# jhidalgocarrio/slam-localization

Hardware: NVIDIA B200
Metric: filter-steps/sec (predict+update) (higher is better)
Workload: dtype f64

## Files before the change

slam-localization_b200/csrc/slb_predict12.cuh:

```cuda
#pragma once
#include "slb_internal.h"
#include "slb_models.cuh"
#include "slb_ptx.cuh"

namespace slbd {

template <int N_>
struct CycCfg {
    static constexpr int N = N_;
    static constexpr int RT = (N_ + 3) / 4;
    static constexpr int CT = (N_ + 7) / 8;
    SLB_HD static constexpr int cb(int k) { return k * N_ - k * (k - 1) / 2; }
    SLB_HD static constexpr bool exists(int r, int c) { return 4 * r < N_ && 8 * c < N_ && 4 * r + 3 >= 8 * c; }
    SLB_HD static constexpr bool live(int k, int r, int c) { return exists(r, c) && 8 * c + 7 > k && 4 * r + 3 > k; }
    SLB_HD static constexpr bool row_live(int k, int r) {
        for (int c = 0; c < CT; ++c)
            if (live(k, r, c)) return true;
        return false;
    }
    SLB_HD static constexpr bool col_live(int k, int c) {
        for (int r = 0; r < RT; ++r)
            if (live(k, r, c)) return true;
        return false;
    }
};

template <class C, int K>
struct CholStep {
    template <class Tile>
    SLB_DEV static void run(Tile &T, double *Ls, int a_, int b_, bool &ok, double x, double nrcp) {
        constexpr int N = C::N, RT = C::RT, CT = C::CT;
        constexpr int rk = K >> 2, bk = K & 7, ck = K >> 3;
        constexpr int K1 = K + 1 < N ? K + 1 : K;
        constexpr int owner1 = (K1 & 3) + 4 * (K1 & 7);
        constexpr int base = C::cb(K) - K;
        ok = ok && (x > 0.0);
        const double xn_old = __shfl_sync(FULL, T[K1 >> 2][K1 >> 3], owner1);
#pragma unroll
        for (int r = rk; r < RT; ++r) {
            const int i = a_ + 4 * r;
            if (b_ == bk && i >= K && i < N) Ls[base + i] = T[r][ck];
        }
        __syncwarp();
        double li[RT], lj[CT];
#pragma unroll
        for (int r = 0; r < RT; ++r)
            if (C::row_live(K, r)) li[r] = Ls[base + a_ + 4 * r];
#pragma unroll
        for (int c = 0; c < CT; ++c)
            if (C::col_live(K, c)) lj[c] = Ls[base + b_ + 8 * c] * nrcp;
        double xn = x, nrcpn = nrcp;
        if (K + 1 < N) {
            const double u1 = Ls[base + K + 1];
            xn = fma(u1, u1 * nrcp, xn_old);
            nrcpn = -rcp_fast(xn);
        }
#pragma unroll
        for (int r = 0; r < RT; ++r)
#pragma unroll
            for (int c = 0; c < CT; ++c)
                if (C::live(K, r, c)) T[r][c] = fma(li[r], lj[c], T[r][c]);
        CholStep<C, K + 1>::run(T, Ls, a_, b_, ok, xn, nrcpn);
    }
};
template <class C>
struct CholStep<C, C::N> {
    template <class Tile>
    SLB_DEV static void run(Tile &, double *, int, int, bool &, double, double) {}
};

constexpr int PRED_DS = 20;
constexpr int PRED_LS = 78 + 16;
constexpr int PRED_D = 28 * PRED_DS;
constexpr int PRED_W = 144;
constexpr int PRED_FK = 12 * PRED_DS;
constexpr int PRED_RSD = 16;
constexpr int PRED_SLOTS = 16;
constexpr int PRED_SCR = PRED_LS + PRED_D + PRED_W + PRED_FK + PRED_RSD + PRED_SLOTS;
constexpr int PRED_PR = 520;
constexpr int PRED_PF = 8 * 12;
constexpr int PRED_MU = 26;
constexpr int PRED_SM = PRED_PR + PRED_PF + PRED_SCR + PRED_MU + 2;
static_assert(16 * PRED_SM * 8 <= 227 * 1024, "two CTAs of 8 warps per SM");

SLB_DEV void load_q_entries(const double *Qi, int a_, int b_, double *qv) {
    const int rr[6] = {b_, b_, 8 + b_, 8 + b_, 8 + b_, 8 + b_};
    const int cc[6] = {2 * a_, 2 * a_ + 1, 2 * a_, 2 * a_ + 1, 8 + 2 * a_, 9 + 2 * a_};
#pragma unroll
    for (int k = 0; k < 6; ++k) qv[k] = (rr[k] < 12 && cc[k] <= rr[k]) ? __ldg(Qi + rr[k] * 12 + cc[k]) : 0.0;
}

SLB_DEV void warp_sum12(const double *v, double *out, double *slots, int lane) {
    double a[8], b[4], c[2], d1;
    const bool h16 = lane & 16, h8 = lane & 8, h4 = lane & 4, h2 = lane & 2;
#pragma unroll
    for (int i = 0; i < 8; ++i) {
        const double lo = v[i], hi = i < 4 ? v[8 + i] : 0.0;
        const double r = __shfl_xor_sync(FULL, h16 ? lo : hi, 16);
        a[i] = (h16 ? hi : lo) + r;
    }
#pragma unroll
    for (int i = 0; i < 4; ++i) {
        const double r = __shfl_xor_sync(FULL, h8 ? a[i] : a[4 + i], 8);
        b[i] = (h8 ? a[4 + i] : a[i]) + r;
    }
#pragma unroll
    for (int i = 0; i < 2; ++i) {
        const double r = __shfl_xor_sync(FULL, h4 ? b[i] : b[2 + i], 4);
        c[i] = (h4 ? b[2 + i] : b[i]) + r;
    }
    {
        const double r = __shfl_xor_sync(FULL, h2 ? c[0] : c[1], 2);
        d1 = (h2 ? c[1] : c[0]) + r;
    }
    d1 += __shfl_xor_sync(FULL, d1, 1);
    const int idx = (h16 ? 8 : 0) + (h8 ? 4 : 0) + (h4 ? 2 : 0) + (h2 ? 1 : 0);
    __syncwarp();
    if (!(lane & 1)) slots[idx] = d1;
    __syncwarp();
#pragma unroll
    for (int i = 0; i < 6; ++i) {
        const double2 t = *reinterpret_cast<const double2 *>(slots + 2 * i);
        out[2 * i] = t.x;
        out[2 * i + 1] = t.y;
    }
}

template <int PM, bool CROSS, bool PIN, class View>
SLB_DEV int predict12_block(View v, const double *mu_src, const double *u, double dt, double *scr, const double *Qg,
                            const double *qv, int nf, double *mu_dst, int lane, bool &dirty) {
    typedef LayState12 L;
    typedef CycCfg<12> C;
    constexpr int ROW0 = View::ROW0;
    double *Ls = scr, *D = Ls + PRED_LS, *W = D + PRED_D, *Fk = W + PRED_W, *rsd = Fk + PRED_FK, *slots = rsd + PRED_RSD;
    const int a_ = lane & 3, b_ = lane >> 2;
    double mu[13];
#pragma unroll
    for (int c = 0; c < 13; ++c) mu[c] = mu_src[c];
    ProcessModel<PM> f;
    f.prepare(u, dt);
    double T[C::RT][C::CT];
#pragma unroll
    for (int r = 0; r < C::RT; ++r)
#pragma unroll
        for (int c = 0; c < C::CT; ++c)
            if (C::exists(r, c)) {
                const int i = a_ + 4 * r, j = b_ + 8 * c;
                T[r][c] = (i < 12 && j <= i) ? v.at(i, ROW0 + j) : 0.0;
            }
    bool ok = true;
    {
        const double x0 = __shfl_sync(FULL, T[0][0], 0);
        CholStep<C, 0>::run(T, Ls, a_, b_, ok, x0, -rcp_fast(x0));
    }
    if (!ok) return SLB_ST_CHOL_FAIL;
    __syncwarp();
    if (lane < 12) {
        double sq_, rs_;
        sqrt_rsqrt(Ls[C::cb(lane)], sq_, rs_);
        rsd[lane] = rs_;
    }
    __syncwarp();
    const bool act = lane < 25;
    const int j = lane >= 1 ? (lane - 1) >> 1 : 0, jc = j < 12 ? j : 11;
    double Y[13];
    {
        const double sgn = (lane & 1) ? rsd[jc] : -rsd[jc];
        const int cj = C::cb(jc) - jc;
        double d[12], X[13];
#pragma unroll
        for (int r = 0; r < 12; ++r) d[r] = (act && lane >= 1 && r >= jc) ? sgn * Ls[cj + r] : 0.0;
        boxplus<L>(mu, d, 1.0, X);
        f.apply(X, Y);
    }
    double ref[13];
#pragma unroll
    for (int c = 0; c < 13; ++c) ref[c] = bcast(Y[c], 0);
    int it = 0;
    double nrm2;
    do {
        double dd[12], md[12], nr[13];
        boxminus<L>(Y, ref, dd);
#pragma unroll
        for (int r = 0; r < 12; ++r) dd[r] = act ? dd[r] : 0.0;
        warp_sum12(dd, md, slots, lane);
        nrm2 = 0.0;
#pragma unroll
        for (int r = 0; r < 12; ++r) {
            md[r] *= (1.0 / 25.0);
            nrm2 += md[r] * md[r];
        }
        boxplus<L>(ref, md, 1.0, nr);
#pragma unroll
        for (int c = 0; c < 13; ++c) ref[c] = nr[c];
    } while (sqrt(nrm2) > 1e-6 && ++it < 10000);
    int st = (it >= 10000) ? SLB_ST_MEAN_NOCONV : 0;
    {
        double dY[12];
        boxminus<L>(Y, ref, dY);
        if (lane < 28) {
#pragma unroll
            for (int r = 0; r < 12; r += 2)
                *reinterpret_cast<double2 *>(D + lane * PRED_DS + r) = act ? make_double2(dY[r], dY[r + 1]) : make_double2(0.0, 0.0);
        }
    }
    __syncwarp();
    dirty = true;
    {
        double c00[2] = {0.0, 0.0}, c10[2] = {0.0, 0.0}, c11[2] = {0.0, 0.0};
        const double *p0 = D + a_ * PRED_DS + b_, *p1 = p0 + 8;
#pragma unroll
        for (int k0 = 0; k0 < 28; k0 += 4) {
            const double f0 = p0[k0 * PRED_DS], f1 = p1[k0 * PRED_DS];
            dmma884(c00[0], c00[1], f0, f0);
            dmma884(c10[0], c10[1], f1, f0);
            dmma884(c11[0], c11[1], f1, f1);
        }
        if (CROSS) {
            for (int e = lane; e < 144; e += 32) {
                const int jj = e / 12, c = e - jj * 12;
                W[e] = 0.5 * (D[(1 + 2 * jj) * PRED_DS + c] - D[(2 + 2 * jj) * PRED_DS + c]);
            }
            __syncwarp();
        }
        auto put = [&](int r, int c, double x, int k) {
            if (r < 12 && c <= r) v.at(r, ROW0 + c) = 0.5 * x + (PIN ? qv[k] : __ldg(Qg + r * 12 + c));
        };
        const int r = b_, c = 2 * a_;
        put(r, c, c00[0], 0); put(r, c + 1, c00[1], 1);
        put(8 + r, c, c10[0], 2); put(8 + r, c + 1, c10[1], 3);
        put(8 + r, 8 + c, c11[0], 4); put(8 + r, 8 + c + 1, c11[1], 5);
    }
    if constexpr (CROSS) {
        if (lane < 12) {
            double x[12];
#pragma unroll
            for (int r = 11; r >= 0; --r) {
                double sacc = 0.0;
#pragma unroll
                for (int p = r + 1; p < 12; ++p) sacc = fma(Ls[C::cb(r) - r + p], x[p], sacc);
                const double rs = rsd[r];
                x[r] = (W[r * 12 + lane] - rs * sacc) * rs;
            }
#pragma unroll
            for (int r = 0; r < 12; ++r) Fk[lane * PRED_DS + r] = x[r];
        }
        __syncwarp();
        double oc[2][3][2];
        {
            const int r0 = min(b_, 11), r1 = min(8 + b_, 11);
#pragma unroll
            for (int I = 0; I < 2; ++I)
#pragma unroll
                for (int J = 0; J < 3; ++J) oc[I][J][0] = oc[I][J][1] = 0.0;
#pragma unroll
            for (int k0 = 0; k0 < 12; k0 += 4) {
                const double fa0 = Fk[r0 * PRED_DS + k0 + a_], fa1 = Fk[r1 * PRED_DS + k0 + a_];
#pragma unroll
                for (int J = 0; J < 3; ++J) {
                    const double bv = v.at(k0 + a_, 8 * J + b_);
                    dmma884(oc[0][J][0], oc[0][J][1], fa0, bv);
                    dmma884(oc[1][J][0], oc[1][J][1], fa1, bv);
                }
            }
        }
        const int nft = (nf + 7) >> 3;
        double of[4][2][2];
        {
            const int c0 = min(b_, 11), c1 = min(8 + b_, 11);
#pragma unroll
            for (int I = 0; I < 4; ++I) {
                if (I < nft) {
                    of[I][0][0] = of[I][0][1] = of[I][1][0] = of[I][1][1] = 0.0;
                    const int fr = min(8 * I + b_, nf - 1);
#pragma unroll
                    for (int k0 = 0; k0 < 12; k0 += 4) {
                        const double av = v.feat(fr, k0 + a_);
                        dmma884(of[I][0][0], of[I][0][1], av, Fk[c0 * PRED_DS + k0 + a_]);
                        dmma884(of[I][1][0], of[I][1][1], av, Fk[c1 * PRED_DS + k0 + a_]);
                    }
                }
            }
        }
        __syncwarp();
#pragma unroll
        for (int I = 0; I < 2; ++I)
#pragma unroll
            for (int J = 0; J < 3; ++J)
                if (8 * I + b_ < 12)
                    *reinterpret_cast<double2 *>(v.P + v.idx(8 * I, 8 * J) + 2 * lane) = make_double2(oc[I][J][0], oc[I][J][1]);
#pragma unroll
        for (int I = 0; I < 4; ++I) {
            if (I < nft) {
#pragma unroll
                for (int J = 0; J < 2; ++J) {
                    const int fr = 8 * I + b_, c = 8 * J + 2 * a_;
                    if (fr < nf && c < 12) { v.feat(fr, c) = of[I][J][0]; v.feat(fr, c + 1) = of[I][J][1]; }
                }
            }
        }
    }
    bool finite = true;
#pragma unroll
    for (int c = 0; c < 13; ++c) {
        finite = finite && isfinite(ref[c]);
        if (lane == c) mu_dst[c] = ref[c];
    }
    if (!finite) st |= SLB_ST_NONFINITE;
    __syncwarp();
    return st;
}

struct SpanView {
    static constexpr int ROW0 = 24;
    double *P, *Pf;
    int N;
    SLB_DEV int idx(int r, int c) const { return prec(N, 24 + r, c) - tri(24, 0); }
    SLB_DEV double &at(int r, int c) const { return P[idx(r, c)]; }
    SLB_DEV double &feat(int fr, int c) const { return fr < 4 ? at(12 + fr, 24 + c) : Pf[(fr - 4) * 12 + c]; }
};
template <int ROW0_>
struct PackedView {
    static constexpr int ROW0 = ROW0_;
    double *P;
    SLB_DEV int idx(int r, int c) const { return tri(ROW0 + r, c) - tri(ROW0, 0); }
    SLB_DEV double &at(int r, int c) const { return P[idx(r, c)]; }
};

template <int PM, int WPB, int ROW0, int MU0, bool CROSS, bool PIN = false>
__global__ void __launch_bounds__(WPB * 32, 2) predict12_kernel(slb::FilterArgs a) {
    extern __shared__ __align__(16) double smem[];
    const int lane = threadIdx.x & 31, w = threadIdx.x >> 5;
    const int inst = blockIdx.x * WPB + w;
    if (inst >= a.B) return;
    double *Pr = smem + (size_t)w * PRED_SM, *Pf = Pr + PRED_PR, *scr = Pf + PRED_PF;
    double *mus = scr + PRED_SCR, *us = mus + 13;
    uint64_t *bar = reinterpret_cast<uint64_t *>(mus + PRED_MU);
    static_assert(!CROSS || ROW0 == 24, "the tiled span is tile rows 3..4");
    const int nf = CROSS ? a.nk + a.nl : 0, N = CROSS ? 36 + nf : ROW0 + 12;
    constexpr int T0 = ROW0 * (ROW0 + 1) / 2, T1 = (ROW0 + 12) * (ROW0 + 13) / 2;
    constexpr int RS = CROSS ? 40 : ROW0 + 12;
    constexpr int NFS = RS - 36;
    const int SPAN = CROSS ? tri(min(N, RS), 0) - T0 : T1 - T0;
    const int nfr = CROSS && nf > NFS ? nf - NFS : 0;
    static_assert(tri(RS, 0) - T0 <= PRED_PR && (!CROSS || 12 * (48 - RS) <= PRED_PF), "row span");
    double *Pg = a.P + (size_t)inst * a.pstride;
    double *mug = a.mu + (size_t)inst * a.qstride;
    const int a_ = lane & 3, b_ = lane >> 2;

    static_assert((T0 * 8) % 16 == 0 && ((T1 - T0) * 8) % 16 == 0 && PRED_SM % 2 == 0 &&
                      (!CROSS || (((tri(RS, 0) - T0) * 8) % 16 == 0 && ((tri(39, 0) - T0) * 8) % 16 == 0)),
                  "bulk copy needs 16-byte alignment");
    if (lane == 0) {
        mbar_init(bar, 1);
        mbar_expect_tx(bar, SPAN * 8);
        bulk_g2s(Pr, Pg + T0, SPAN * 8, bar);
    }
    for (int e = lane; e < nfr * 12; e += 32) {
        const int r = e / 12, c = e - r * 12;
        cp_async8(Pf + e, Pg + prec(N, RS + r, 24 + c));
    }
    double qv[PIN ? 6 : 1];
    if (PIN) load_q_entries(a.Q + (size_t)inst * a.qs, a_, b_, qv);
    static_assert(ProcessModel<PM>::NU <= PRED_MU - 13, "control input slots");
    if (lane < 13) cp_async8(mus + lane, mug + MU0 + lane);
    if (lane < ProcessModel<PM>::NU) cp_async8(us + lane, a.u + (size_t)inst * ProcessModel<PM>::NU + lane);
    cp_async_wait_all();
    __syncwarp();
    mbar_wait(bar, 0);

    int st;
    bool dirty = false;
    if constexpr (CROSS) st = predict12_block<PM, true, PIN>(SpanView{Pr, Pf, N}, mus, us, a.dt, scr, a.Q, qv, nf, mug + MU0, lane, dirty);
    else st = predict12_block<PM, false, PIN>(PackedView<ROW0>{Pr}, mus, us, a.dt, scr, a.Q, qv, nf, mug + MU0, lane, dirty);
    if (dirty) {
        for (int e = lane; e < SPAN; e += 32) Pg[T0 + e] = Pr[e];
        for (int e = lane; e < nfr * 12; e += 32) {
            const int r = e / 12, c = e - r * 12;
            Pg[prec(N, RS + r, 24 + c)] = Pf[e];
        }
    }
    if (st && lane == 0) a.status[inst] |= st;
}

}
```

slam-localization_b200/csrc/slb_usckf_step.cuh:

```cuda
#pragma once
#include "slb_predict12.cuh"

#ifndef SLB_USCKF_CTA_SYNC
#define SLB_USCKF_CTA_SYNC 0
#endif
#if SLB_USCKF_CTA_SYNC
#define SLB_CTA_SYNC() __syncthreads()
#else
#define SLB_CTA_SYNC() ((void)0)
#endif

namespace slbd {

template <int NK_, int NL_>
struct StepCfg {
    static constexpr int NK = NK_, NL = NL_, NF = NK_ + NL_;
    static constexpr int N = 36 + NK_ + NL_;
    static constexpr int NP = N * (N + 1) / 2;
    static constexpr int PSTR = (NP + 15) / 16 * 16;
    static constexpr int QD = 39 + NK_ + NL_;
    static constexpr int QS = (QD + 1) / 2 * 2;
    static constexpr int NT = (N + 7) / 8;
    static constexpr int NPAD = 8 * NT;
    static constexpr int JM = 36 + NK_;
    static constexpr int NPAN = (JM + 3) / 4;
    static constexpr int NCOL = 4 * NPAN;
    static constexpr int JLAST = (NCOL - 1) >> 3;
    static constexpr int NGRP = (NPAN + 3) / 4;
    static constexpr int PL = 2 * NPAD + 8;
    static constexpr int PS4 = 2 * PL + 2;
    static constexpr int KP = (NK_ + 3) / 4 * 4;
    static constexpr int NTN = (NK_ + 7) / 8;
    static constexpr int LF = 4 * PS4;
    static constexpr int LRAW = 2 * PL;
    static constexpr int KK = 2 * NPAD * KP + NPAD;
    static constexpr int SCR0 = (LF + LRAW > KK ? LF + LRAW : KK);
    static constexpr int WS = 20;
    static constexpr int WGS = WS * NK_;
    static constexpr int UPD_SCR = SCR0 + WGS + NPAD;
    static constexpr int SCR = (UPD_SCR > PRED_SCR ? UPD_SCR : PRED_SCR);
    static constexpr int ZS = (NK_ + 1) / 2 * 2;
    static constexpr int SM = PSTR + QS + SCR + ZS + 2;
    static constexpr int RP = (NK_ * (NK_ + 1) / 2 + 1) / 2 * 2;
    static constexpr int SMP = SM + RP;
    static_assert(NK_ % 3 == 0 && NK_ >= 3, "the VO model moves 3-D features");
    static_assert(N <= 64, "two rows per lane");
    static_assert(SM % 2 == 0 && PSTR % 2 == 0 && QS % 2 == 0, "16-byte alignment of the bulk copies");
};

template <int M>
SLB_DEV bool sym_inverse(const double *S, double *Si) {
    double L[M * (M + 1) / 2], dd[M], rd[M];
    bool ok = true;
#pragma unroll
    for (int k = 0; k < M; ++k) {
        double d = S[tri(k, k)];
#pragma unroll
        for (int p = 0; p < k; ++p) d = fma(-L[tri(k, p)] * L[tri(k, p)], dd[p], d);
        ok = ok && (d > 0.0);
        dd[k] = d;
        rd[k] = rcp_fast(d);
#pragma unroll
        for (int i = k + 1; i < M; ++i) {
            double s = S[tri(i, k)];
#pragma unroll
            for (int p = 0; p < k; ++p) s = fma(-L[tri(i, p)] * L[tri(k, p)], dd[p], s);
            L[tri(i, k)] = s * rd[k];
        }
    }
    double X[M * (M + 1) / 2];
#pragma unroll
    for (int j = 0; j < M; ++j) {
        X[tri(j, j)] = 1.0;
#pragma unroll
        for (int i = j + 1; i < M; ++i) {
            double s = 0.0;
#pragma unroll
            for (int p = j; p < i; ++p) s = fma(-L[tri(i, p)], X[tri(p, j)], s);
            X[tri(i, j)] = s;
        }
    }
#pragma unroll
    for (int i = 0; i < M; ++i)
#pragma unroll
        for (int j = 0; j <= i; ++j) {
            double s = 0.0;
#pragma unroll
            for (int k = i; k < M; ++k) s = fma(X[tri(k, i)] * rd[k], X[tri(k, j)], s);
            Si[tri(i, j)] = s;
        }
    return ok;
}

template <int NK>
SLB_DEV void vo_model(const double *pk, const double *qk, const double *pi, const double *qi, const double *f, double *z) {
    double dq[4];
    quat_cmul(qi, qk, dq);
#pragma unroll
    for (int c = 0; c < NK; c += 3) {
        double rz[3];
        rotmat_apply(dq, f + c, rz);
        z[c] = rz[0] + (pk[0] - pi[0]);
        z[c + 1] = rz[1] + (pk[1] - pi[1]);
        z[c + 2] = rz[2] + (pk[2] - pi[2]);
    }
}

template <class C>
struct UpdState {
    double c0[C::NT][C::JLAST + 1], c1[C::NT][C::JLAST + 1];
    double x0[C::NT][C::NTN], x1[C::NT][C::NTN];
    double esum[C::NK], eep[C::NK * (C::NK + 1) / 2];
    double z0[C::NK];
    bool ok;
};

template <class C, int G>
SLB_DEV void sigma_group(UpdState<C> &s, const double *mus_, const double *Lf, double *Wg, const double *dv, int lane) {
    constexpr int NK = C::NK, PS4 = C::PS4;
    double mus[40 + NK];
    {
        const double2 *m2 = reinterpret_cast<const double2 *>(mus_);
#pragma unroll
        for (int e = 0; e < 4; ++e) { const double2 v = m2[e]; mus[2 * e] = v.x; mus[2 * e + 1] = v.y; }
#pragma unroll
        for (int e = 13; e < 17; ++e) { const double2 v = m2[e]; mus[2 * e] = v.x; mus[2 * e + 1] = v.y; }
#pragma unroll
        for (int c = 0; c < NK; ++c) mus[39 + c] = mus_[39 + c];
    }
    constexpr int col0 = 16 * G;
    constexpr int ncols = C::NCOL - col0 < 16 ? C::NCOL - col0 : 16;
    const bool neg = lane & 1, act = (lane >> 1) < ncols;
    const int jl = act ? lane >> 1 : 0;
    const double rs = rsqrt_fast(dv[col0 + jl]);
    const double sgn = act ? (neg ? -rs : rs) : 0.0;
    constexpr int RW = 8 * ((col0 + ncols - 1) >> 3);
    const double *col = Lf + (jl >> 2) * PS4 + ((jl & 3) >> 1) * C::PL + (jl & 1);
    auto Lc = [&](int r) -> double { return sgn * (r >= RW || r >= col0 + jl ? col[2 * r] : 0.0); };
    double xpk[3], xqk[4], xpi[3], xqi[4], xf[NK];
    if (col0 <= 5) {
#pragma unroll
        for (int c = 0; c < 3; ++c) xpk[c] = mus[c] + Lc(c);
        const double v[3] = {Lc(3), Lc(4), Lc(5)};
        const double q[4] = {mus[3], mus[4], mus[5], mus[6]};
        double e[4];
        so3_exp(v, 1.0, e);
        quat_mul(q, e, xqk);
    } else {
#pragma unroll
        for (int c = 0; c < 3; ++c) xpk[c] = mus[c];
#pragma unroll
        for (int c = 0; c < 4; ++c) xqk[c] = mus[3 + c];
    }
    if (col0 <= 29) {
#pragma unroll
        for (int c = 0; c < 3; ++c) xpi[c] = mus[26 + c] + Lc(24 + c);
        const double v[3] = {Lc(27), Lc(28), Lc(29)};
        const double q[4] = {mus[29], mus[30], mus[31], mus[32]};
        double e[4];
        so3_exp(v, 1.0, e);
        quat_mul(q, e, xqi);
    } else {
#pragma unroll
        for (int c = 0; c < 3; ++c) xpi[c] = mus[26 + c];
#pragma unroll
        for (int c = 0; c < 4; ++c) xqi[c] = mus[29 + c];
    }
#pragma unroll
    for (int c = 0; c < NK; ++c) xf[c] = mus[39 + c] + Lc(36 + c);
    double z[NK];
    vo_model<NK>(xpk, xqk, xpi, xqi, xf, z);
    double e[NK];
#pragma unroll
    for (int c = 0; c < NK; ++c) {
        e[c] = act ? z[c] - s.z0[c] : 0.0;
        s.esum[c] += e[c];
        const double zp = __shfl_xor_sync(FULL, z[c], 1);
        if (act && !neg) Wg[c * C::WS + jl] = (0.5 * rs) * (z[c] - zp);
    }
#pragma unroll
    for (int r = 0; r < NK; ++r)
#pragma unroll
        for (int c = 0; c <= r; ++c) s.eep[tri(r, c)] = fma(e[r], e[c], s.eep[tri(r, c)]);
    __syncwarp();
    const int a_ = lane & 3, b_ = lane >> 2;
#pragma unroll
    for (int qq = 0; qq < ncols / 4; ++qq) {
        const int J0 = (col0 + 4 * qq) >> 3;
        const double *fp = Lf + qq * PS4 + (a_ >> 1) * C::PL + (a_ & 1) + 2 * b_;
        double w[C::NTN];
#pragma unroll
        for (int T = 0; T < C::NTN; ++T) w[T] = 8 * T + b_ < NK ? Wg[(8 * T + b_) * C::WS + 4 * qq + a_] : 0.0;
#pragma unroll
        for (int I = J0; I < C::NT; ++I) {
            const double f = fp[16 * I];
#pragma unroll
            for (int T = 0; T < C::NTN; ++T) dmma884(s.x0[I][T], s.x1[I][T], f, w[T]);
        }
    }
}

template <class C, int P>
struct PanelStep {
    SLB_DEV static void run(UpdState<C> &s, const double *mus, double *Lf, double *Lraw, double *Wg, double *dv, int lane) {
        constexpr int NT = C::NT, JLAST = C::JLAST, PS4 = C::PS4;
        constexpr int K = 4 * P, J0 = K >> 3, H = (K >> 2) & 1, Q = P & 3;
        constexpr int I1 = (K + 4) >> 3;
        const int a_ = lane & 3, b_ = lane >> 2;
        double *Lq = Lf + Q * PS4;
        constexpr int PL = C::PL;
        if ((a_ >> 1) == H) {
#pragma unroll
            for (int I = J0; I < NT; ++I)
                *reinterpret_cast<double2 *>(Lraw + (a_ & 1) * PL + 2 * (8 * I + b_)) = make_double2(s.c0[I][J0], s.c1[I][J0]);
        }
        __syncwarp();
        double m10, m20, m30, m21, m31, m32, r0, r1, r2, r3, d0, d1, d2, d3;
        {
            const double *A = Lraw + 2 * K, *Bp = A + PL;
            const double a00 = A[0];
            const double2 a1 = *reinterpret_cast<const double2 *>(A + 2);
            const double2 a2 = *reinterpret_cast<const double2 *>(A + 4);
            const double a22 = Bp[4];
            const double2 a3 = *reinterpret_cast<const double2 *>(A + 6), a3b = *reinterpret_cast<const double2 *>(Bp + 6);
            d0 = a00;
            r0 = rcp_fast(d0);
            m10 = a1.x * r0; m20 = a2.x * r0; m30 = a3.x * r0;
            d1 = fma(-a1.x, m10, a1.y);
            const double u21 = fma(-a2.x, m10, a2.y), u31 = fma(-a3.x, m10, a3.y);
            r1 = rcp_fast(d1);
            m21 = u21 * r1; m31 = u31 * r1;
            d2 = fma(-u21, m21, fma(-a2.x, m20, a22));
            const double u32 = fma(-u31, m21, fma(-a3.x, m20, a3b.x));
            r2 = rcp_fast(d2);
            m32 = u32 * r2;
            d3 = fma(-u32, m32, fma(-u31, m31, fma(-a3.x, m30, a3b.y)));
            r3 = rcp_fast(d3);
            s.ok = s.ok && (d0 > 0.0) && (d1 > 0.0) && (d2 > 0.0) && (d3 > 0.0);
        }
        if (lane == 0) {
            *reinterpret_cast<double2 *>(dv + K) = make_double2(d0, d1);
            *reinterpret_cast<double2 *>(dv + K + 2) = make_double2(d2, d3);
        }
        constexpr int R0 = 8 * J0, NLIVE = C::NPAD - R0;
        auto finish = [&](int i) {
            const double2 x01 = *reinterpret_cast<const double2 *>(Lraw + 2 * i);
            const double2 x23 = *reinterpret_cast<const double2 *>(Lraw + PL + 2 * i);
            const double u0 = x01.x;
            const double u1 = fma(-u0, m10, x01.y);
            const double u2 = fma(-u1, m21, fma(-u0, m20, x23.x));
            const double u3 = fma(-u2, m32, fma(-u1, m31, fma(-u0, m30, x23.y)));
            double2 u01, u23;
            u01.x = i >= K ? u0 : 0.0;
            u01.y = i >= K + 1 ? u1 : 0.0;
            u23.x = i >= K + 2 ? u2 : 0.0;
            u23.y = i >= K + 3 ? u3 : 0.0;
            *reinterpret_cast<double2 *>(Lq + 2 * i) = u01;
            *reinterpret_cast<double2 *>(Lq + PL + 2 * i) = u23;
        };
        if (NLIVE >= 32 || lane < NLIVE) finish(R0 + lane);
        if (NLIVE > 32 && lane < NLIVE - 32) finish(R0 + 32 + lane);
        __syncwarp();
        if (I1 <= JLAST) {
            double f[NT];
            const double *fp = Lq + (a_ >> 1) * PL + (a_ & 1) + 2 * b_;
#pragma unroll
            for (int I = I1; I < NT; ++I) f[I] = fp[16 * I];
            const double rlo = (a_ & 1) ? r1 : r0, rhi = (a_ & 1) ? r3 : r2;
            const double nr = -((a_ & 2) ? rhi : rlo);
#pragma unroll
            for (int J = I1; J <= JLAST; ++J) {
                const double g = f[J] * nr;
#pragma unroll
                for (int I = J; I < NT; ++I) dmma884(s.c0[I][J], s.c1[I][J], f[I], g);
            }
        }
        if (Q == 3 || P == C::NPAN - 1) {
            sigma_group<C, (P >> 2)>(s, mus, Lf, Wg, dv, lane);
            SLB_CTA_SYNC();
        }
        PanelStep<C, P + 1>::run(s, mus, Lf, Lraw, Wg, dv, lane);
    }
};
template <class C>
struct PanelStep<C, C::NPAN> {
    SLB_DEV static void run(UpdState<C> &, const double *, double *, double *, double *, double *, int) {}
};

template <int NK, int NL, bool PIN = false>
SLB_DEV int usckf_update_smem(double *Ps, double *mus, double *scr, const double *zs, const double *Rs,
                              const slb::FilterArgs &a, int lane, bool &dirty, double &m2out) {
    typedef StepCfg<NK, NL> C;
    constexpr int N = C::N, NT = C::NT, NPAD = C::NPAD, JLAST = C::JLAST, KP = C::KP;
    const int a_ = lane & 3, b_ = lane >> 2;
    double *Lf = scr, *Lraw = scr + C::LF, *Ks = scr, *Cs = scr + NPAD * KP, *Wg = scr + C::SCR0, *dv = Wg + C::WGS,
           *dl = Cs + NPAD * KP;
    UpdState<C> s;
    s.ok = true;
    auto elem = [&](int i, int j) -> double {
        if (i >= N || j >= N) return i == j ? 1.0 : 0.0;
        return i >= j ? Ps[prec(N, i, j)] : Ps[prec(N, j, i)];
    };
#pragma unroll
    for (int I = 0; I < NT; ++I)
#pragma unroll
        for (int J = 0; J <= JLAST; ++J)
            if (J < I) {
                double2 v = make_double2(0.0, 0.0);
                if (8 * I + b_ < N) v = *reinterpret_cast<const double2 *>(Ps + prec(N, 8 * I, 8 * J) + 2 * lane);
                s.c0[I][J] = v.x;
                s.c1[I][J] = v.y;
            } else if (J == I) {
                const int i = 8 * I + b_, j = 8 * J + 2 * a_;
                s.c0[I][J] = elem(i, j);
                s.c1[I][J] = elem(i, j + 1);
            }
#pragma unroll
    for (int I = 0; I < NT; ++I)
#pragma unroll
        for (int T = 0; T < C::NTN; ++T) s.x0[I][T] = s.x1[I][T] = 0.0;
#pragma unroll
    for (int c = 0; c < NK; ++c) s.esum[c] = 0.0;
#pragma unroll
    for (int e = 0; e < NK * (NK + 1) / 2; ++e) s.eep[e] = 0.0;
    {
        double pk[3], qk[4], pi[3], qi[4], ft[NK];
#pragma unroll
        for (int c = 0; c < 3; ++c) { pk[c] = mus[c]; pi[c] = mus[26 + c]; }
#pragma unroll
        for (int c = 0; c < 4; ++c) { qk[c] = mus[3 + c]; qi[c] = mus[29 + c]; }
#pragma unroll
        for (int c = 0; c < NK; ++c) ft[c] = mus[39 + c];
        vo_model<NK>(pk, qk, pi, qi, ft, s.z0);
    }
    PanelStep<C, 0>::run(s, mus, Lf, Lraw, Wg, dv, lane);
    if (!s.ok) return SLB_ST_CHOL_FAIL;

    constexpr double NS = (double)(2 * N + 1);
    double ebar[NK], S[NK * (NK + 1) / 2];
    if (PIN) {
        cp_async_wait0();
        __syncwarp();
    }
    auto Rv = [&](int r, int c) { return PIN ? Rs[tri(r, c)] : __ldg(a.R + r * NK + c); };
    if (NK == 3) {
        double v[12], o[12];
#pragma unroll
        for (int c = 0; c < 3; ++c) v[c] = s.esum[c];
#pragma unroll
        for (int e = 0; e < 6; ++e) v[3 + e] = s.eep[e];
        v[9] = v[10] = v[11] = 0.0;
        warp_sum12(v, o, dv, lane);
#pragma unroll
        for (int c = 0; c < 3; ++c) ebar[c] = o[c] * (1.0 / NS);
#pragma unroll
        for (int r = 0; r < NK; ++r)
#pragma unroll
            for (int c = 0; c <= r; ++c)
                S[tri(r, c)] = 0.5 * fma(-NS * ebar[r], ebar[c], o[3 + tri(r, c)]) + Rv(r, c);
    } else {
#pragma unroll
        for (int c = 0; c < NK; ++c) ebar[c] = warp_sum(s.esum[c]) * (1.0 / NS);
#pragma unroll
        for (int r = 0; r < NK; ++r)
#pragma unroll
            for (int c = 0; c <= r; ++c)
                S[tri(r, c)] = 0.5 * fma(-NS * ebar[r], ebar[c], warp_sum(s.eep[tri(r, c)])) + Rv(r, c);
    }
    double Si[NK * (NK + 1) / 2];
    const bool sok = sym_inverse<NK>(S, Si);
    auto SiAt = [&](int r, int c) { return r >= c ? Si[tri(r, c)] : Si[tri(c, r)]; };
    cp_async_wait0();
    __syncwarp();
    double nu[NK], sn[NK], m2 = 0.0;
#pragma unroll
    for (int c = 0; c < NK; ++c) nu[c] = zs[c] - (s.z0[c] + ebar[c]);
#pragma unroll
    for (int r = 0; r < NK; ++r) {
        double t = 0.0;
#pragma unroll
        for (int c = 0; c < NK; ++c) t = fma(SiAt(r, c), nu[c], t);
        sn[r] = t;
        m2 = fma(nu[r], t, m2);
    }
    if (!sok) return SLB_ST_CHOL_FAIL;
    m2out = m2;
    if (!chi2_accept(m2, a.gate)) return SLB_ST_GATE_REJECT;
#pragma unroll
    for (int I = 0; I < NT; ++I)
#pragma unroll
        for (int T = 0; T < C::NTN; ++T)
            if (8 * T + 2 * a_ < KP)
                *reinterpret_cast<double2 *>(Cs + (8 * I + b_) * KP + 8 * T + 2 * a_) = make_double2(s.x0[I][T], s.x1[I][T]);
    __syncwarp();
    auto finish_row = [&](int i) {
        double px[NK];
#pragma unroll
        for (int c = 0; c < NK; ++c) px[c] = Cs[i * KP + c];
        double dsum = 0.0;
#pragma unroll
        for (int c = 0; c < KP; ++c) {
            double k = 0.0;
            if (c < NK) {
#pragma unroll
                for (int p = 0; p < NK; ++p) k = fma(px[p], SiAt(p, c), k);
                dsum = fma(px[c], sn[c], dsum);
            }
            Ks[i * KP + c] = k;
            Cs[i * KP + c] = c < NK ? -px[c] : 0.0;
        }
        dl[i] = dsum;
    };
    finish_row(lane);
    if (lane + 32 < NPAD) finish_row(lane + 32);
    __syncwarp();
    dirty = true;
    bool finite = true;
    if (lane < 12) {
        const int mbw = lane & 3;
        const int mqo = 13 * (lane >> 2) + (mbw == 0 ? 0 : mbw == 1 ? 3 : mbw == 2 ? 7 : 10);
        const double v[3] = {dl[3 * lane], dl[3 * lane + 1], dl[3 * lane + 2]};
        if (mbw == 1) {
            const double q[4] = {mus[mqo], mus[mqo + 1], mus[mqo + 2], mus[mqo + 3]};
            double e[4], o[4];
            so3_exp(v, 1.0, e);
            quat_mul(q, e, o);
#pragma unroll
            for (int c = 0; c < 4; ++c) { mus[mqo + c] = o[c]; finite = finite && isfinite(o[c]); }
        } else {
#pragma unroll
            for (int c = 0; c < 3; ++c) {
                const double o = mus[mqo + c] + v[c];
                mus[mqo + c] = o;
                finite = finite && isfinite(o);
            }
        }
    }
    for (int f = lane; f < NK + NL; f += 32) {
        const double o = mus[39 + f] + dl[36 + f];
        mus[39 + f] = o;
        finite = finite && isfinite(o);
    }
    {
        double fa[NT][KP / 4], fb[NT][KP / 4];
#pragma unroll
        for (int I = 0; I < NT; ++I)
#pragma unroll
            for (int kk = 0; kk < KP / 4; ++kk) {
                fa[I][kk] = Cs[(8 * I + b_) * KP + 4 * kk + a_];
                fb[I][kk] = Ks[(8 * I + b_) * KP + 4 * kk + a_];
            }
#pragma unroll
        for (int I = 0; I < NT; ++I)
#pragma unroll
            for (int J = 0; J <= I; ++J) {
                const int i = 8 * I + b_, j = 8 * J + 2 * a_;
                if (J < I) {
                    double2 *pp = reinterpret_cast<double2 *>(Ps + prec(N, 8 * I, 8 * J) + 2 * lane);
                    const bool w = i < N;
                    double2 p = w ? *pp : make_double2(0.0, 0.0);
#pragma unroll
                    for (int kk = 0; kk < KP / 4; ++kk) dmma884(p.x, p.y, fa[I][kk], fb[J][kk]);
                    if (w) *pp = p;
                } else {
                    const bool w0 = i < N && j <= i, w1 = i < N && j + 1 <= i;
                    double p0 = w0 ? Ps[prec(N, i, j)] : 0.0, p1 = w1 ? Ps[prec(N, i, j + 1)] : 0.0;
#pragma unroll
                    for (int kk = 0; kk < KP / 4; ++kk) dmma884(p0, p1, fa[I][kk], fb[J][kk]);
                    if (w0) Ps[prec(N, i, j)] = p0;
                    if (w1) Ps[prec(N, i, j + 1)] = p1;
                }
            }
    }
    return __all_sync(FULL, finite) ? 0 : SLB_ST_NONFINITE;
}

template <int N>
struct ResidentView {
    static constexpr int ROW0 = 24;
    double *P;
    SLB_DEV int idx(int r, int c) const { return prec(N, 24 + r, c); }
    SLB_DEV double &at(int r, int c) const { return P[idx(r, c)]; }
    SLB_DEV double &feat(int fr, int c) const { return P[prec(N, 36 + fr, 24 + c)]; }
};

template <int PM, int NK, int NL, bool PRED, bool UPD, int WPB, int MINB, bool PIN = false, bool NIS = false>
__global__ void __launch_bounds__(WPB * 32, MINB) usckf_step_kernel(slb::FilterArgs a) {
    typedef StepCfg<NK, NL> C;
    constexpr int SMW = PIN ? C::SMP : C::SM;
    extern __shared__ __align__(128) double smem[];
    const int lane = threadIdx.x & 31, w = threadIdx.x >> 5;
    const int inst = blockIdx.x * WPB + w;
    if (inst >= a.B) return;
    double *Ps = smem + (size_t)w * SMW, *mus = Ps + C::PSTR, *scr = mus + C::QS, *zs = scr + C::SCR;
    double *Rs = zs + C::ZS;
    uint64_t *bar = reinterpret_cast<uint64_t *>(zs + C::ZS + (PIN ? C::RP : 0));
    double *Pg = a.P + (size_t)inst * a.pstride;
    double *mug = a.mu + (size_t)inst * a.qstride;
    if (lane == 0) {
        mbar_init(bar, 1);
        mbar_expect_tx(bar, (C::PSTR + C::QS) * 8);
        bulk_g2s(Ps, Pg, C::PSTR * 8, bar);
        bulk_g2s(mus, mug, C::QS * 8, bar);
        if (a.prefetch > 0 && inst + a.prefetch < a.B) bulk_prefetch_l2(Pg + (size_t)a.prefetch * a.pstride, C::PSTR * 8);
    }
    if (UPD && lane < NK) {
        cp_async8(zs + lane, a.z + (size_t)inst * NK + lane);
        cp_async_commit();
    }
    if (PIN && UPD) {
        const double *Ri = a.R + (size_t)inst * a.rs;
        for (int e = lane; e < NK * (NK + 1) / 2; e += 32) {
            int r = (int)((sqrtf(8.0f * e + 1.0f) - 1.0f) * 0.5f);
            r += (tri(r + 1, 0) <= e) - (tri(r, 0) > e);
            cp_async8(Rs + e, Ri + r * NK + (e - tri(r, 0)));
        }
        cp_async_commit();
    }
    double qv[PIN && PRED ? 6 : 1];
    if (PIN && PRED) load_q_entries(a.Q + (size_t)inst * a.qs, lane & 3, lane >> 2, qv);
    double u[ProcessModel<PM>::NU];
    if (PRED) {
#pragma unroll
        for (int c = 0; c < ProcessModel<PM>::NU; ++c) u[c] = a.u[(size_t)inst * ProcessModel<PM>::NU + c];
    }
    __syncwarp();
    mbar_wait(bar, 0);
    SLB_CTA_SYNC();
    int st = 0;
    bool dirty = false;
    if (PRED) {
        st = predict12_block<PM, true, PIN>(ResidentView<C::N>{Ps}, mus + 26, u, a.dt, scr, a.Q, qv, NK + NL, mus + 26, lane, dirty);
    }
    if (PRED) SLB_CTA_SYNC();
    double m2 = __longlong_as_double(0x7ff8000000000000ll);
    if (UPD) st |= usckf_update_smem<NK, NL, PIN>(Ps, mus, scr, zs, Rs, a, lane, dirty, m2);
    if (NIS && lane == 0) a.nis[inst] = m2;
    cp_async_wait0();
    if (dirty) {
        fence_proxy_async();
        __syncwarp();
        if (lane == 0) bulk_s2g(Pg, Ps, C::PSTR * 8);
        for (int e = lane; e < C::QD; e += 32) mug[e] = mus[e];
    }
    if (a.mu_out) {
        __syncwarp();
        for (int e = lane; e < a.out_len; e += 32) a.mu_out[(size_t)inst * a.out_len + e] = mus[a.out_off + e];
    }
    if (st && lane == 0) a.status[inst] |= st;
    if (dirty && lane == 0) bulk_store_wait();
}

}
```

Baseline: 101.5 million.

## Replace predict's scalar 12x12 Cholesky with blocked 4-wide panels using DMMA updates

The predict-stage 12x12 factorisation is rewritten from a fully unrolled rank-1 step per column (shuffle plus shared-memory broadcast per step) into three 4-column panel steps. Each panel does a small scalar factorisation and then a trailing update through dmma884 tensor-core FP64 MMAs, reusing the panel code shared with the update kernel (factored into a Panel4 helper). The panel is parked in the D scratch region, and padded rows are filled with identity. This reduces the number of warp sync steps, at the cost of padding waste and extra shared-memory traffic for this small matrix.

Result: slower. 100.1 million, median of 6 (-1.3%).

```diff
diff --git a/profiles/predict_share.py b/profiles/predict_share.py
--- /dev/null
+++ b/profiles/predict_share.py
@@ -0,0 +1,83 @@
+import argparse
+import json
+import os
+import subprocess
+import sys
+
+import numpy as np
+
+ROOT = os.path.dirname(os.path.dirname(os.path.abspath(__file__)))
+sys.path.insert(0, ROOT)
+
+ARMS = ("predict", "update", "predict+update", "step")
+
+
+def card():
+    q = "name,power.limit,clocks.sm,clocks.max.sm"
+    out = subprocess.run(["nvidia-smi", "--query-gpu=" + q, "--format=csv,noheader", "-i", "0"], capture_output=True,
+                         text=True).stdout.strip()
+    return dict(zip(q.split(","), [x.strip() for x in out.split(",")]))
+
+
+def main():
+    ap = argparse.ArgumentParser()
+    ap.add_argument("--steps", type=int, default=200)
+    ap.add_argument("--warmup", type=int, default=5)
+    ap.add_argument("--reps", type=int, default=3)
+    ap.add_argument("--tag", default="", help="free-form label copied into every line (e.g. the tree)")
+    ap.add_argument("--out", default=None)
+    args = ap.parse_args()
+    import torch
+    if not torch.cuda.is_available():
+        sys.exit("predict_share.py needs a CUDA device (no CPU fallback)")
+    from slam_localization_b200 import engine, synth
+    info = card()
+    B, npri, seed = 524288, 2048, 4321
+    sc = synth.usckf_scenario(npri, seed=seed + 1)
+    rng = np.random.default_rng(seed + 1)
+    rep = B // npri
+    u = np.concatenate([rng.normal(size=(B, 3)), rng.normal(size=(B, 3)) * 0.2], axis=1)
+    z = np.tile(sc["mu"][:, 39:42], (rep, 1)) + rng.normal(size=(B, 3)) * 0.1
+    f = engine.Usckf(B, nk=3, nl=9)
+    du, dz = engine.DeviceArray(u), engine.DeviceArray(z)
+    Q, R = engine.DeviceArray(sc["Q"]), engine.DeviceArray(sc["R"])
+    pm, mm, dt = engine.PM_USCKF_TEST, engine.MM_USCKF_VO, sc["dt"]
+    calls = {
+        "predict": lambda: f.predict(pm, du, dt, Q),
+        "update": lambda: f.update(mm, dz, R),
+        "predict+update": lambda: (f.predict(pm, du, dt, Q), f.update(mm, dz, R)),
+        "step": lambda: f.step(pm, mm, du, dt, Q, dz, R),
+    }
+    lines = []
+    for r in range(args.reps):
+        for arm in ARMS:
+            f.set_state(sc["mu"], sc["P"], replicate=True)
+            for _ in range(args.warmup):
+                calls[arm]()
+            torch.cuda.synchronize()
+            e0, e1 = torch.cuda.Event(enable_timing=True), torch.cuda.Event(enable_timing=True)
+            e0.record()
+            for _ in range(args.steps):
+                calls[arm]()
+            e1.record()
+            torch.cuda.synchronize()
+            ms = e0.elapsed_time(e1) / args.steps
+            line = dict(tag=args.tag, arm=arm, run=r + 1, instances=B, nk=3, nl=9, steps=args.steps, ms=ms,
+                        status_counts=f.status_counts(), lib=os.environ.get("SLB_LIB", "in-tree"), card=info)
+            print(json.dumps(line), flush=True)
+            lines.append(line)
+    med = {}
+    for arm in ARMS:
+        v = sorted(x["ms"] for x in lines if x["arm"] == arm)
+        med[arm] = v[len(v) // 2]
+        print("# %-14s median %.4f ms  spread %.4f ms (%d runs)" % (arm, med[arm], v[-1] - v[0], len(v)))
+    print("# predict / (predict + update) = %.3f;  predict + update - step = %.4f ms"
+          % (med["predict"] / (med["predict"] + med["update"]), med["predict+update"] - med["step"]))
+    if args.out:
+        with open(args.out, "a") as fo:
+            for x in lines:
+                fo.write(json.dumps(x) + "\n")
+
+
+if __name__ == "__main__":
+    main()
diff --git a/slam-localization_b200/csrc/slb_predict12.cuh b/slam-localization_b200/csrc/slb_predict12.cuh
--- a/slam-localization_b200/csrc/slb_predict12.cuh
+++ b/slam-localization_b200/csrc/slb_predict12.cuh
@@ -5,78 +5,50 @@
 
 namespace slbd {
 
-template <int N_>
-struct CycCfg {
-    static constexpr int N = N_;
-    static constexpr int RT = (N_ + 3) / 4;
-    static constexpr int CT = (N_ + 7) / 8;
-    SLB_HD static constexpr int cb(int k) { return k * N_ - k * (k - 1) / 2; }
-    SLB_HD static constexpr bool exists(int r, int c) { return 4 * r < N_ && 8 * c < N_ && 4 * r + 3 >= 8 * c; }
-    SLB_HD static constexpr bool live(int k, int r, int c) { return exists(r, c) && 8 * c + 7 > k && 4 * r + 3 > k; }
-    SLB_HD static constexpr bool row_live(int k, int r) {
-        for (int c = 0; c < CT; ++c)
-            if (live(k, r, c)) return true;
-        return false;
-    }
-    SLB_HD static constexpr bool col_live(int k, int c) {
-        for (int r = 0; r < RT; ++r)
-            if (live(k, r, c)) return true;
-        return false;
-    }
-};
-
-template <class C, int K>
-struct CholStep {
-    template <class Tile>
-    SLB_DEV static void run(Tile &T, double *Ls, int a_, int b_, bool &ok, double x, double nrcp) {
-        constexpr int N = C::N, RT = C::RT, CT = C::CT;
-        constexpr int rk = K >> 2, bk = K & 7, ck = K >> 3;
-        constexpr int K1 = K + 1 < N ? K + 1 : K;
-        constexpr int owner1 = (K1 & 3) + 4 * (K1 & 7);
-        constexpr int base = C::cb(K) - K;
-        ok = ok && (x > 0.0);
-        const double xn_old = __shfl_sync(FULL, T[K1 >> 2][K1 >> 3], owner1);
-#pragma unroll
-        for (int r = rk; r < RT; ++r) {
-            const int i = a_ + 4 * r;
-            if (b_ == bk && i >= K && i < N) Ls[base + i] = T[r][ck];
-        }
-        __syncwarp();
-        double li[RT], lj[CT];
-#pragma unroll
-        for (int r = 0; r < RT; ++r)
-            if (C::row_live(K, r)) li[r] = Ls[base + a_ + 4 * r];
-#pragma unroll
-        for (int c = 0; c < CT; ++c)
-            if (C::col_live(K, c)) lj[c] = Ls[base + b_ + 8 * c] * nrcp;
-        double xn = x, nrcpn = nrcp;
-        if (K + 1 < N) {
-            const double u1 = Ls[base + K + 1];
-            xn = fma(u1, u1 * nrcp, xn_old);
-            nrcpn = -rcp_fast(xn);
-        }
-#pragma unroll
-        for (int r = 0; r < RT; ++r)
-#pragma unroll
-            for (int c = 0; c < CT; ++c)
-                if (C::live(K, r, c)) T[r][c] = fma(li[r], lj[c], T[r][c]);
-        CholStep<C, K + 1>::run(T, Ls, a_, b_, ok, xn, nrcpn);
-    }
-};
-template <class C>
-struct CholStep<C, C::N> {
-    template <class Tile>
-    SLB_DEV static void run(Tile &, double *, int, int, bool &, double, double) {}
+struct Panel4 {
+    double m10, m20, m30, m21, m31, m32, r0, r1, r2, r3, d0, d1, d2, d3;
+    SLB_DEV Panel4(const double *A, int PL) {
+        const double *Bp = A + PL;
+        const double a00 = A[0];
+        const double2 a1 = *reinterpret_cast<const double2 *>(A + 2);
+        const double2 a2 = *reinterpret_cast<const double2 *>(A + 4);
+        const double a22 = Bp[4];
+        const double2 a3 = *reinterpret_cast<const double2 *>(A + 6), a3b = *reinterpret_cast<const double2 *>(Bp + 6);
+        d0 = a00;
+        r0 = rcp_fast(d0);
+        m10 = a1.x * r0; m20 = a2.x * r0; m30 = a3.x * r0;
+        d1 = fma(-a1.x, m10, a1.y);
+        const double u21 = fma(-a2.x, m10, a2.y), u31 = fma(-a3.x, m10, a3.y);
+        r1 = rcp_fast(d1);
+        m21 = u21 * r1; m31 = u31 * r1;
+        d2 = fma(-u21, m21, fma(-a2.x, m20, a22));
+        const double u32 = fma(-u31, m21, fma(-a3.x, m20, a3b.x));
+        r2 = rcp_fast(d2);
+        m32 = u32 * r2;
+        d3 = fma(-u32, m32, fma(-u31, m31, fma(-a3.x, m30, a3b.y)));
+        r3 = rcp_fast(d3);
+    }
+    SLB_DEV bool ok() const { return (d0 > 0.0) && (d1 > 0.0) && (d2 > 0.0) && (d3 > 0.0); }
+    SLB_DEV void row(const double *Lraw, int PL, int i, double (&u)[4]) const {
+        const double2 x01 = *reinterpret_cast<const double2 *>(Lraw + 2 * i);
+        const double2 x23 = *reinterpret_cast<const double2 *>(Lraw + PL + 2 * i);
+        u[0] = x01.x;
+        u[1] = fma(-u[0], m10, x01.y);
+        u[2] = fma(-u[1], m21, fma(-u[0], m20, x23.x));
+        u[3] = fma(-u[2], m32, fma(-u[1], m31, fma(-u[0], m30, x23.y)));
+    }
 };
 
 constexpr int PRED_DS = 20;
 constexpr int PRED_LS = 78 + 16;
+constexpr int PRED_PL = 2 * 16 + 8;
 constexpr int PRED_D = 28 * PRED_DS;
 constexpr int PRED_W = 144;
 constexpr int PRED_FK = 12 * PRED_DS;
 constexpr int PRED_RSD = 16;
 constexpr int PRED_SLOTS = 16;
 constexpr int PRED_SCR = PRED_LS + PRED_D + PRED_W + PRED_FK + PRED_RSD + PRED_SLOTS;
+static_assert(2 * PRED_PL <= PRED_D, "the parked panel lives in D, dead until the deviations are written");
 constexpr int PRED_PR = 520;
 constexpr int PRED_PF = 8 * 12;
 constexpr int PRED_MU = 26;
@@ -126,11 +98,51 @@
     }
 }
 
+SLB_HD constexpr int cb12(int k) { return k * 12 - k * (k - 1) / 2; }
+
+template <int P>
+SLB_DEV void pred_panel(double (&c0)[2][2], double (&c1)[2][2], double *Ls, double *Lraw, int lane, bool &ok) {
+    constexpr int K = 4 * P, J0 = K >> 3, H = P & 1, I1 = (K + 4) >> 3, R0 = 8 * J0;
+    const int a_ = lane & 3, b_ = lane >> 2;
+    if ((a_ >> 1) == H) {
+#pragma unroll
+        for (int I = J0; I < 2; ++I)
+            *reinterpret_cast<double2 *>(Lraw + (a_ & 1) * PRED_PL + 2 * (8 * I + b_)) = make_double2(c0[I][J0], c1[I][J0]);
+    }
+    __syncwarp();
+    const Panel4 p(Lraw + 2 * K, PRED_PL);
+    ok = ok && p.ok();
+    if (lane < 12 - R0) {
+        const int i = R0 + lane;
+        double uu[4];
+        p.row(Lraw, PRED_PL, i, uu);
+#pragma unroll
+        for (int c = 0; c < 4; ++c)
+            if (i >= K + c) Ls[cb12(K + c) - (K + c) + i] = uu[c];
+    }
+    if (P < 2) {
+        __syncwarp();
+        double fr[2];
+#pragma unroll
+        for (int I = I1; I < 2; ++I) {
+            const int i = 8 * I + b_, k = K + a_;
+            fr[I] = (i >= k && i < 12) ? Ls[cb12(k) - k + i] : 0.0;
+        }
+        const double rlo = (a_ & 1) ? p.r1 : p.r0, rhi = (a_ & 1) ? p.r3 : p.r2;
+        const double nr = -((a_ & 2) ? rhi : rlo);
+#pragma unroll
+        for (int J = I1; J < 2; ++J) {
+            const double g = fr[J] * nr;
+#pragma unroll
+            for (int I = J; I < 2; ++I) dmma884(c0[I][J], c1[I][J], fr[I], g);
+        }
+    }
+}
+
 template <int PM, bool CROSS, bool PIN, class View>
 SLB_DEV int predict12_block(View v, const double *mu_src, const double *u, double dt, double *scr, const double *Qg,
                             const double *qv, int nf, double *mu_dst, int lane, bool &dirty) {
     typedef LayState12 L;
-    typedef CycCfg<12> C;
     constexpr int ROW0 = View::ROW0;
     double *Ls = scr, *D = Ls + PRED_LS, *W = D + PRED_D, *Fk = W + PRED_W, *rsd = Fk + PRED_FK, *slots = rsd + PRED_RSD;
     const int a_ = lane & 3, b_ = lane >> 2;
@@ -139,25 +151,35 @@
     for (int c = 0; c < 13; ++c) mu[c] = mu_src[c];
     ProcessModel<PM> f;
     f.prepare(u, dt);
-    double T[C::RT][C::CT];
-#pragma unroll
-    for (int r = 0; r < C::RT; ++r)
-#pragma unroll
-        for (int c = 0; c < C::CT; ++c)
-            if (C::exists(r, c)) {
-                const int i = a_ + 4 * r, j = b_ + 8 * c;
-                T[r][c] = (i < 12 && j <= i) ? v.at(i, ROW0 + j) : 0.0;
-            }
+    double c0[2][2], c1[2][2];
+    {
+        auto elem = [&](int i, int j) -> double {
+            if (i >= 12) return i == j ? 1.0 : 0.0;
+            return j <= i ? v.at(i, ROW0 + j) : 0.0;
+        };
+        c0[0][0] = elem(b_, 2 * a_);
+        c1[0][0] = elem(b_, 2 * a_ + 1);
+        c0[1][1] = elem(8 + b_, 8 + 2 * a_);
+        c1[1][1] = elem(8 + b_, 9 + 2 * a_);
+        if (CROSS) {
+            double2 t = make_double2(0.0, 0.0);
+            if (b_ < 4) t = *reinterpret_cast<const double2 *>(v.P + v.idx(8, ROW0) + 2 * lane);
+            c0[1][0] = t.x;
+            c1[1][0] = t.y;
+        } else {
+            c0[1][0] = b_ < 4 ? v.at(8 + b_, ROW0 + 2 * a_) : 0.0;
+            c1[1][0] = b_ < 4 ? v.at(8 + b_, ROW0 + 2 * a_ + 1) : 0.0;
+        }
+    }
     bool ok = true;
-    {
-        const double x0 = __shfl_sync(FULL, T[0][0], 0);
-        CholStep<C, 0>::run(T, Ls, a_, b_, ok, x0, -rcp_fast(x0));
-    }
+    pred_panel<0>(c0, c1, Ls, D, lane, ok);
+    pred_panel<1>(c0, c1, Ls, D, lane, ok);
+    pred_panel<2>(c0, c1, Ls, D, lane, ok);
     if (!ok) return SLB_ST_CHOL_FAIL;
     __syncwarp();
     if (lane < 12) {
         double sq_, rs_;
-        sqrt_rsqrt(Ls[C::cb(lane)], sq_, rs_);
+        sqrt_rsqrt(Ls[cb12(lane)], sq_, rs_);
         rsd[lane] = rs_;
     }
     __syncwarp();
@@ -166,7 +188,7 @@
     double Y[13];
     {
         const double sgn = (lane & 1) ? rsd[jc] : -rsd[jc];
-        const int cj = C::cb(jc) - jc;
+        const int cj = cb12(jc) - jc;
         double d[12], X[13];
 #pragma unroll
         for (int r = 0; r < 12; ++r) d[r] = (act && lane >= 1 && r >= jc) ? sgn * Ls[cj + r] : 0.0;
@@ -238,7 +260,7 @@
             for (int r = 11; r >= 0; --r) {
                 double sacc = 0.0;
 #pragma unroll
-                for (int p = r + 1; p < 12; ++p) sacc = fma(Ls[C::cb(r) - r + p], x[p], sacc);
+                for (int p = r + 1; p < 12; ++p) sacc = fma(Ls[cb12(r) - r + p], x[p], sacc);
                 const double rs = rsd[r];
                 x[r] = (W[r * 12 + lane] - rs * sacc) * rs;
             }
diff --git a/slam-localization_b200/csrc/slb_usckf_step.cuh b/slam-localization_b200/csrc/slb_usckf_step.cuh
--- a/slam-localization_b200/csrc/slb_usckf_step.cuh
+++ b/slam-localization_b200/csrc/slb_usckf_step.cuh
@@ -215,46 +215,21 @@
                 *reinterpret_cast<double2 *>(Lraw + (a_ & 1) * PL + 2 * (8 * I + b_)) = make_double2(s.c0[I][J0], s.c1[I][J0]);
         }
         __syncwarp();
-        double m10, m20, m30, m21, m31, m32, r0, r1, r2, r3, d0, d1, d2, d3;
-        {
-            const double *A = Lraw + 2 * K, *Bp = A + PL;
-            const double a00 = A[0];
-            const double2 a1 = *reinterpret_cast<const double2 *>(A + 2);
-            const double2 a2 = *reinterpret_cast<const double2 *>(A + 4);
-            const double a22 = Bp[4];
-            const double2 a3 = *reinterpret_cast<const double2 *>(A + 6), a3b = *reinterpret_cast<const double2 *>(Bp + 6);
-            d0 = a00;
-            r0 = rcp_fast(d0);
-            m10 = a1.x * r0; m20 = a2.x * r0; m30 = a3.x * r0;
-            d1 = fma(-a1.x, m10, a1.y);
-            const double u21 = fma(-a2.x, m10, a2.y), u31 = fma(-a3.x, m10, a3.y);
-            r1 = rcp_fast(d1);
-            m21 = u21 * r1; m31 = u31 * r1;
-            d2 = fma(-u21, m21, fma(-a2.x, m20, a22));
-            const double u32 = fma(-u31, m21, fma(-a3.x, m20, a3b.x));
-            r2 = rcp_fast(d2);
-            m32 = u32 * r2;
-            d3 = fma(-u32, m32, fma(-u31, m31, fma(-a3.x, m30, a3b.y)));
-            r3 = rcp_fast(d3);
-            s.ok = s.ok && (d0 > 0.0) && (d1 > 0.0) && (d2 > 0.0) && (d3 > 0.0);
-        }
+        const Panel4 p(Lraw + 2 * K, PL);
+        s.ok = s.ok && p.ok();
         if (lane == 0) {
-            *reinterpret_cast<double2 *>(dv + K) = make_double2(d0, d1);
-            *reinterpret_cast<double2 *>(dv + K + 2) = make_double2(d2, d3);
+            *reinterpret_cast<double2 *>(dv + K) = make_double2(p.d0, p.d1);
+            *reinterpret_cast<double2 *>(dv + K + 2) = make_double2(p.d2, p.d3);
         }
         constexpr int R0 = 8 * J0, NLIVE = C::NPAD - R0;
         auto finish = [&](int i) {
-            const double2 x01 = *reinterpret_cast<const double2 *>(Lraw + 2 * i);
-            const double2 x23 = *reinterpret_cast<const double2 *>(Lraw + PL + 2 * i);
-            const double u0 = x01.x;
-            const double u1 = fma(-u0, m10, x01.y);
-            const double u2 = fma(-u1, m21, fma(-u0, m20, x23.x));
-            const double u3 = fma(-u2, m32, fma(-u1, m31, fma(-u0, m30, x23.y)));
+            double u[4];
+            p.row(Lraw, PL, i, u);
             double2 u01, u23;
-            u01.x = i >= K ? u0 : 0.0;
-            u01.y = i >= K + 1 ? u1 : 0.0;
-            u23.x = i >= K + 2 ? u2 : 0.0;
-            u23.y = i >= K + 3 ? u3 : 0.0;
+            u01.x = i >= K ? u[0] : 0.0;
+            u01.y = i >= K + 1 ? u[1] : 0.0;
+            u23.x = i >= K + 2 ? u[2] : 0.0;
+            u23.y = i >= K + 3 ? u[3] : 0.0;
             *reinterpret_cast<double2 *>(Lq + 2 * i) = u01;
             *reinterpret_cast<double2 *>(Lq + PL + 2 * i) = u23;
         };
@@ -266,7 +241,7 @@
             const double *fp = Lq + (a_ >> 1) * PL + (a_ & 1) + 2 * b_;
 #pragma unroll
             for (int I = I1; I < NT; ++I) f[I] = fp[16 * I];
-            const double rlo = (a_ & 1) ? r1 : r0, rhi = (a_ & 1) ? r3 : r2;
+            const double rlo = (a_ & 1) ? p.r1 : p.r0, rhi = (a_ & 1) ? p.r3 : p.r2;
             const double nr = -((a_ & 2) ? rhi : rlo);
 #pragma unroll
             for (int J = I1; J <= JLAST; ++J) {
```
